# ilyamaclean/microclimf

Hardware: AMD Instinct MI355X
Metric: cell-steps/s (higher is better)
Workload: dtype f64

## Files before the change

### include/mcf.h

```cpp
#ifndef MCF_H
#define MCF_H

#include <stdint.h>

#ifdef __cplusplus
extern "C" {
#endif

#define MCF_ABI_VERSION 8

enum {
    MCF_OUT_TZ = 0,
    MCF_OUT_TLEAF = 1,
    MCF_OUT_RELHUM = 2,
    MCF_OUT_SOILM = 3,
    MCF_OUT_WINDSPEED = 4,
    MCF_OUT_RDIRDOWN = 5,
    MCF_OUT_RDIFDOWN = 6,
    MCF_OUT_RLWDOWN = 7,
    MCF_OUT_RSWUP = 8,
    MCF_OUT_RLWUP = 9,
    MCF_NOUT = 10
};

// ... 138 lines not shown
} mcf_nc_spec;
typedef struct mcf_ncfile mcf_ncfile;
int mcf_nc_create(const char *path, const mcf_nc_spec *spec, mcf_ncfile **nc);
int mcf_nc_write_host(mcf_ncfile *nc, int64_t step0, int64_t nsteps, const double *const vars[MCF_NOUT]);
int mcf_nc_write_plan(mcf_ncfile *nc, mcf_plan *plan, int32_t slot, int64_t slot_step0, int64_t file_step0,
                      int64_t nsteps, float *kernel_ms);
int mcf_nc_close(mcf_ncfile *nc);

int mcf_plan_slot_ptr(mcf_plan *plan, int32_t slot, int32_t var, void **dev_ptr);
typedef struct mcf_ring_layout {
    int32_t tiled;
    int32_t cells_per_tile;
    int32_t block_doubles;
    int32_t slot_days;
    int64_t cells;
    int64_t tile_stride;
    int64_t day_stride;
} mcf_ring_layout;
int mcf_plan_ring_layout(mcf_plan *plan, mcf_ring_layout *layout);
int64_t mcf_ring_index(const mcf_ring_layout *layout, int64_t cell, int64_t step);

int mcf_plan_timer_start(mcf_plan *plan);
int mcf_plan_timer_stop(mcf_plan *plan, float *ms);
int mcf_plan_kernel_timing(mcf_plan *plan, int32_t enable);
int mcf_plan_kernel_stats(mcf_plan *plan, double *total_ms, int64_t *launches);

typedef struct mcf_dispatch_stats {
    int64_t fast_tiles, slow_tiles;
    int64_t irregular_days;
    int64_t fast_launches, slow_launches;
    int64_t canary_trips;
} mcf_dispatch_stats;
int mcf_plan_dispatch_stats(mcf_plan *plan, mcf_dispatch_stats *stats);

#define MCF_NBIO 19
typedef struct mcf_bioclim_sel {
    const int32_t *wetq, *dryq, *hotq, *colq;
    int32_t nwet, ndry, nhot, ncol;
    int32_t air;
    int32_t out[MCF_NBIO];
} mcf_bioclim_sel;
typedef struct mcf_bioclim_out {
    double *bio[MCF_NBIO];
} mcf_bioclim_out;
int mcf_runbioclim1(const mcf_grid_inputs *in, const mcf_options *opt, const mcf_bioclim_sel *sel,
                    mcf_bioclim_out *out);
int mcf_runbioclim2(const mcf_grid_inputs *in, const mcf_options *opt, const mcf_bioclim_sel *sel,
                    mcf_bioclim_out *out);
int mcf_runbioclim3(const mcf_grid_inputs *in, const mcf_options *opt, const mcf_bioclim_sel *sel,
                    mcf_bioclim_out *out);
int mcf_runbioclim4(const mcf_grid_inputs *in, const mcf_options *opt, const mcf_bioclim_sel *sel,
                    mcf_bioclim_out *out);
int mcf_runbioclim1_multi(const mcf_grid_inputs *in, const mcf_options *opt, const mcf_bioclim_sel *sel, const mcf_multi *multi,
                          mcf_bioclim_out *out);
int mcf_runbioclim2_multi(const mcf_grid_inputs *in, const mcf_options *opt, const mcf_bioclim_sel *sel, const mcf_multi *multi,
                          mcf_bioclim_out *out);
int mcf_runbioclim3_multi(const mcf_grid_inputs *in, const mcf_options *opt, const mcf_bioclim_sel *sel, const mcf_multi *multi,
                          mcf_bioclim_out *out);
int mcf_runbioclim4_multi(const mcf_grid_inputs *in, const mcf_options *opt, const mcf_bioclim_sel *sel, const mcf_multi *multi,
                          mcf_bioclim_out *out);

typedef struct mcf_terrain_in {
    int64_t rows, cols;
    int32_t halo_north, halo_south;
    const double *dtm;
    double res;
// ... 216 lines not shown
```

### microclimf_amd/_abi.py

```python
from __future__ import annotations

import ctypes as C
import os
from pathlib import Path

NOUT = 10
OUT_NAMES = ("Tz", "tleaf", "relhum", "soilm", "windspeed", "Rdirdown",
             "Rdifdown", "Rlwdown", "Rswup", "Rlwup")

c_double_p = C.POINTER(C.c_double)
c_int32_p = C.POINTER(C.c_int32)


class Obstime(C.Structure):
    _fields_ = [("year", c_int32_p), ("month", c_int32_p), ("day", c_int32_p),
                ("hour", c_double_p)]


CLIM_FIELDS = ("tc", "es", "ea", "tdew", "pk", "swdown", "difrad", "lwdown",
               "windspeed", "winddir")
POINTM_FIELDS = ("soilm", "Tg", "Tbp", "G", "umu", "kp", "muGp", "dtrp")
VEGP_FIELDS = ("hgt", "pai", "x", "gsmax", "leafr", "leaft", "clump", "leafd",
               "paia", "leafden")
SOILC_FIELDS = ("Smin", "Smax", "gref", "soilb", "Psie", "Vq", "Vm", "Mc", "rho",
# ... 123 lines not shown

class PointSnowOut(C.Structure):
    _fields_ = [(k, c_double_p) for k in POINTSNOW_FIELDS] + [("mxdif", C.c_double), ("iters", C.c_int32)]


class SnowDriverIn(C.Structure):
    _fields_ = [("base", SnowInputs), ("dtm", c_double_p), ("res", C.c_double), ("tfact", C.c_double),
                ("chunk_steps", C.c_int32), ("af_wsa_s", C.c_int32), ("af_wind", c_double_p)]


SNOWDRIVER_OUT = ("Tc", "Tg", "groundsnowdepth", "totalSWE", "snowden")
SnowDriverOut = _ptr_struct("SnowDriverOut", SNOWDRIVER_OUT)


class MicrosnowIn(C.Structure):
    _fields_ = [("grid", C.POINTER(GridInputs)), ("snow", C.POINTER(SnowDriverIn)), ("micro", C.POINTER(SnowInputs)),
                ("mat", C.c_double)]

_PKG_DIR = Path(__file__).resolve().parent
LIB_PATH = _PKG_DIR / "csrc" / "libmcfhip.so"

EXPORTS = (
    "mcf_abi_version", "mcf_last_error", "mcf_device_count",
    "mcf_runmicro1", "mcf_runmicro2", "mcf_runmicro3", "mcf_runmicro4",
    "mcf_plan_create", "mcf_plan_destroy", "mcf_plan_twi_partial",
    "mcf_plan_set_twi_mean", "mcf_plan_upload_forcing_days", "mcf_plan_run_days",
    "mcf_plan_belowground", "mcf_plan_sync", "mcf_plan_fetch", "mcf_plan_fetch_cells", "mcf_plan_fetch_packed", "mcf_plan_slot_ptr",
    "mcf_plan_ring_layout", "mcf_ring_index", "mcf_plan_run_days_at", "mcf_plan_run_days_masked", "mcf_plan_set_mxtc",
    "mcf_snowplan_covered_tiles", "mcf_plan_run_days_cells", "mcf_snowplan_free_cells",
    "mcf_runmicro1_multi", "mcf_runmicro2_multi", "mcf_runmicro3_multi", "mcf_runmicro4_multi", "mcf_plan_fetch_pitched",
    "mcf_snowplan_reset", "mcf_snowplan_checkpoint", "mcf_snowplan_restore", "mcf_snowplan_fetch_cells", "mcf_snowplan_keep_chunk", "mcf_snowplan_can_keep", "mcf_snowplan_set_keep_budget", "mcf_plan_set_mxtc_days", "mcf_snowplan_set_series",
    "mcf_snowplan_release_kept", "mcf_snowplan_meand_accumulate", "mcf_snowplan_micro_setup", "mcf_snowplan_microsnow",
    "mcf_plan_timer_start", "mcf_plan_timer_stop", "mcf_plan_kernel_timing",
    "mcf_plan_kernel_stats", "mcf_plan_dispatch_stats", "mcf_plan_valid_cells", "mcf_plan_bytes", "mcf_selftest_math",
    "mcf_precompute_terrain", "mcf_precompute_terrain_multi", "mcf_runbioclim1_multi", "mcf_runbioclim2_multi",
    "mcf_runbioclim3_multi", "mcf_runbioclim4_multi", "mcf_runbioclim1", "mcf_runbioclim2", "mcf_runbioclim3", "mcf_runbioclim4",
    "mcf_snowenv_from_name", "mcf_gridmodelsnow1", "mcf_gridmodelsnow2", "mcf_gridmicrosnow1",
    "mcf_gridmicrosnow2", "mcf_snowmodel1", "mcf_snowmodel2", "mcf_snowmodel1_multi", "mcf_applycpp3",
    "mcf_snowplan_create", "mcf_snowplan_destroy", "mcf_snowplan_chunks", "mcf_snowplan_surface", "mcf_snowplan_handover", "mcf_snowplan_apply3",
    "mcf_snowplan_surface_partial", "mcf_snowplan_prepare_chunk", "mcf_snowplan_run_chunk", "mcf_snowplan_pack_halo",
    "mcf_snowplan_prepare_chunk_dev",
    "mcf_bigleaf", "mcf_soilm", "mcf_pointmprocess", "mcf_weatherhgt", "mcf_man", "mcf_pointmodelsnow", "mcf_canintfrac", "mcf_meltmu", "mcf_meltmu2", "mcf_tpicalc",
    "mcf_nc_create", "mcf_nc_write_host", "mcf_nc_write_plan", "mcf_nc_close",
    "mcf_flowacc", "mcf_topidx",
    "mcf_runmicrosnow1", "mcf_runmicrosnow2", "mcf_runmicrosnow1_multi", "mcf_snowrun_create", "mcf_snowrun_destroy", "mcf_snowrun_days", "mcf_snowrun_stats", "mcf_snowrun_keep",
    "mcf_snowrun_pass1", "mcf_snowrun_pass2", "mcf_snowplan_run_chunk_pitched", "mcf_snowplan_chunk_af",
    "mcf_plan_create_streamed", "mcf_plan_below_prepare", "mcf_plan_below_set_days", "mcf_below_days_range",
    "mcf_runmicrosnow1_below", "mcf_runmicrosnow1_below_multi", "mcf_snowrun_create_below",
    "mcf_flowacc_device", "mcf_topidx_device", "mcf_plan_create_dtm", "mcf_runmicro_dtm",
)

ABI_VERSION = 8
_lib = None


class McfError(RuntimeError):
    """Raised when libmcfhip reports a non-zero status."""


class DispatchStats(C.Structure):
    _fields_ = [(n, C.c_int64) for n in ("fast_tiles", "slow_tiles", "irregular_days", "fast_launches", "slow_launches",
                                         "canary_trips")]


class RingLayout(C.Structure):
    _fields_ = [("tiled", C.c_int32), ("cells_per_tile", C.c_int32), ("block_doubles", C.c_int32), ("slot_days", C.c_int32),
                ("cells", C.c_int64), ("tile_stride", C.c_int64), ("day_stride", C.c_int64)]
# ... 118 lines not shown
        lib.mcf_plan_below_set_days.argtypes = [P, c_int32_p, C.c_int32]
        lib.mcf_below_days_range.restype = C.c_int
        lib.mcf_below_days_range.argtypes = [c_int32_p, C.c_int32, C.c_int32, C.c_int32, C.c_int32, c_int32_p, c_int32_p]
    lib.mcf_plan_sync.restype = C.c_int
    lib.mcf_plan_sync.argtypes = [P]
    lib.mcf_plan_fetch.restype = C.c_int
    lib.mcf_plan_fetch.argtypes = [P, C.c_int32, C.c_int32, C.c_int64, C.c_int64, c_double_p]
    lib.mcf_plan_fetch_cells.restype = C.c_int
    lib.mcf_plan_fetch_cells.argtypes = [P, C.c_int32, C.c_int32, C.c_int64, C.c_int64, C.POINTER(C.c_int64), C.c_int64,
                                         c_double_p]
    lib.mcf_plan_fetch_packed.restype = C.c_int
    lib.mcf_plan_fetch_packed.argtypes = [P, C.c_int32, C.c_int32, C.c_int64, C.c_int64, C.c_double, c_int32_p,
                                          C.POINTER(C.c_float)]
    lib.mcf_plan_slot_ptr.restype = C.c_int
    lib.mcf_plan_slot_ptr.argtypes = [P, C.c_int32, C.c_int32, C.POINTER(C.c_void_p)]
    try:
        lib.mcf_plan_ring_layout.restype = C.c_int
        lib.mcf_plan_ring_layout.argtypes = [P, C.POINTER(RingLayout)]
        lib.mcf_ring_index.restype = C.c_int64
        lib.mcf_ring_index.argtypes = [C.POINTER(RingLayout), C.c_int64, C.c_int64]
    except AttributeError:
        if "MCF_LIB" not in os.environ:
            raise
    lib.mcf_plan_timer_start.restype = C.c_int
    lib.mcf_plan_timer_start.argtypes = [P]
    lib.mcf_plan_timer_stop.restype = C.c_int
    lib.mcf_plan_timer_stop.argtypes = [P, C.POINTER(C.c_float)]
    lib.mcf_plan_kernel_timing.restype = C.c_int
    lib.mcf_plan_kernel_timing.argtypes = [P, C.c_int32]
    lib.mcf_plan_kernel_stats.restype = C.c_int
    lib.mcf_plan_kernel_stats.argtypes = [P, c_double_p, C.POINTER(C.c_int64)]
    lib.mcf_plan_dispatch_stats.restype = C.c_int
    lib.mcf_plan_dispatch_stats.argtypes = [P, C.POINTER(DispatchStats)]
    lib.mcf_plan_valid_cells.restype = C.c_int64
    lib.mcf_plan_valid_cells.argtypes = [P]
    lib.mcf_plan_bytes.restype = C.c_int64
    lib.mcf_plan_bytes.argtypes = [P]
    lib.mcf_selftest_math.restype = C.c_int
    lib.mcf_selftest_math.argtypes = [C.c_int32, c_double_p, c_double_p, c_double_p, C.c_int64, C.c_int32]
    for fn in (lib.mcf_runbioclim1, lib.mcf_runbioclim2, lib.mcf_runbioclim3, lib.mcf_runbioclim4):
        fn.restype = C.c_int
        fn.argtypes = [GI, OP, C.POINTER(BioclimSel), C.POINTER(BioclimOut)]
    for fn in (lib.mcf_runbioclim1_multi, lib.mcf_runbioclim2_multi, lib.mcf_runbioclim3_multi, lib.mcf_runbioclim4_multi):
        fn.restype = C.c_int
        fn.argtypes = [GI, OP, C.POINTER(BioclimSel), C.POINTER(Multi), C.POINTER(BioclimOut)]
    lib.mcf_snowenv_from_name.restype = C.c_int32
    lib.mcf_snowenv_from_name.argtypes = [C.c_char_p]
    SI = C.POINTER(SnowInputs)
    for fn in (lib.mcf_gridmodelsnow1, lib.mcf_gridmodelsnow2):
        fn.restype = C.c_int
        fn.argtypes = [SI, C.POINTER(SnowModelOut), C.c_int32]
    for fn in (lib.mcf_gridmicrosnow1, lib.mcf_gridmicrosnow2):
        fn.restype = C.c_int
        fn.argtypes = [SI, C.POINTER(Snowm), C.c_double, C.c_double, C.POINTER(C.c_int32 * NOUT), OU, C.c_int32]
    PW, OT = C.POINTER(PointWeather), C.POINTER(Obstime)
    lib.mcf_bigleaf.restype = C.c_int
    lib.mcf_bigleaf.argtypes = [C.c_int64, OT, PW, c_double_p, c_double_p, c_double_p, C.c_double, C.c_double, C.c_double,
                                C.c_double, C.c_int32, C.c_double, C.c_double, C.c_int32, C.POINTER(BigLeafOut)]
    lib.mcf_soilm.restype = C.c_int
    lib.mcf_soilm.argtypes = [C.c_int64, PW] + [C.c_double] * 7 + [c_double_p, C.POINTER(C.c_int64)]
    lib.mcf_pointmprocess.restype = C.c_int
    lib.mcf_pointmprocess.argtypes = [C.c_int64] + [c_double_p] * 7 + [C.c_double] * 7 + [c_double_p] * 6
    lib.mcf_weatherhgt.restype = C.c_int
    lib.mcf_weatherhgt.argtypes = [C.c_int64, OT, PW] + [C.c_double] * 5 + [c_double_p] * 3
    lib.mcf_pointmodelsnow.restype = C.c_int
    lib.mcf_pointmodelsnow.argtypes = [C.c_int64, C.POINTER(Obstime), C.POINTER(PointWeather), c_double_p, c_double_p,
# ... 109 lines not shown
```

### microclimf_amd/api.py

```python
from __future__ import annotations

import ctypes as C
from typing import Mapping, Sequence

import numpy as np

from . import _abi
from .marshal import Marshalled, alloc_outputs, marshal


DTM_DERIVED = ("slope", "aspect", "hor", "svfa", "wsa", "twi")


def dtm_spec(dtm: Mapping, rows: int, cols: int):
    z = np.asfortranarray(np.asarray(dtm["z"], dtype=np.float64))
    hn, hs = int(dtm.get("halo_north", 0)), int(dtm.get("halo_south", 0))
    if z.shape != (hn + rows + hs, cols):
        raise ValueError(f"dtm$z: expected shape {(hn + rows + hs, cols)}, got {z.shape}")
    res = dtm["res"]
    xres, yres = (res, res) if np.isscalar(res) else res
    sp = _abi.DtmSpec()
    sp.dtm = z.ctypes.data_as(_abi.c_double_p)
    sp.halo_north, sp.halo_south = hn, hs
    sp.row0, sp.rows_total = int(dtm.get("row0", 0)), int(dtm.get("rows_total", 0))
# ... 254 lines not shown
    def fetch_packed(self, slot: int, var, step0: int, nsteps: int, scale: float | None = None,
                     timing: bool = False):
        v = _abi.OUT_NAMES.index(var) if isinstance(var, str) else int(var)
        if scale is None:
            scale = self.NC_SCALE[_abi.OUT_NAMES[v]]
        a = np.empty((self.cols, self.rows, nsteps), dtype=np.int32, order="F")
        ms = C.c_float()
        _abi.check(self._lib.mcf_plan_fetch_packed(self._p, slot, v, step0, nsteps, float(scale),
                                                   a.ctypes.data_as(_abi.c_int32_p),
                                                   C.byref(ms) if timing else None))
        return (a, ms.value) if timing else a

    def ring_layout(self) -> dict:
        lay = _abi.RingLayout()
        _abi.check(self._lib.mcf_plan_ring_layout(self._p, C.byref(lay)))
        return {n: int(getattr(lay, n)) for n, _ in lay._fields_}

    def timer_start(self):
        _abi.check(self._lib.mcf_plan_timer_start(self._p))

    def timer_stop(self) -> float:
        ms = C.c_float()
        _abi.check(self._lib.mcf_plan_timer_stop(self._p, C.byref(ms)))
        return ms.value

    def kernel_timing(self, enable: bool = True):
        _abi.check(self._lib.mcf_plan_kernel_timing(self._p, 1 if enable else 0))

    def dispatch_stats(self) -> dict:
        st = _abi.DispatchStats()
        _abi.check(self._lib.mcf_plan_dispatch_stats(self._p, C.byref(st)))
        return {n: int(getattr(st, n)) for n, _ in st._fields_}

    def kernel_stats(self):
        ms, n = C.c_double(), C.c_int64()
        _abi.check(self._lib.mcf_plan_kernel_stats(self._p, C.byref(ms), C.byref(n)))
        return ms.value, n.value


def below_days_range(days, total_days: int, day0: int, ndays: int):
    d = np.ascontiguousarray(np.asarray(days).astype(np.int32))
    pos0, npos = C.c_int32(), C.c_int32()
    _abi.check(_abi.load().mcf_below_days_range(d.ctypes.data_as(_abi.c_int32_p), int(d.size), int(total_days), int(day0), int(ndays),
                                                C.byref(pos0), C.byref(npos)))
    return pos0.value, npos.value


def runbioclim3Cpp(obstime, climdata, pointm, vegp, soilc, reqhgt, zref, lat, lon, Sminp, Smaxp, tfact, mat, out,
                   wetq, dryq, hotq, colq, air, *, device: int = 0, devices=None, n_blocks: int = 0) -> dict:
    return _bioclim("mcf_runbioclim3", False, obstime, climdata, pointm, vegp, soilc, reqhgt, zref, lat, lon,
                    Sminp, Smaxp, tfact, mat, out, wetq, dryq, hotq, colq, air, device, True, devices=devices, n_blocks=n_blocks)


def runbioclim4Cpp(obstime, climdata, pointm, vegp, soilc, reqhgt, zref, lats, lons, Sminp, Smaxp, tfact, mat, out,
                   wetq, dryq, hotq, colq, air, *, device: int = 0, devices=None, n_blocks: int = 0) -> dict:
    return _bioclim("mcf_runbioclim4", True, obstime, climdata, pointm, vegp, soilc, reqhgt, zref, lats, lons,
                    Sminp, Smaxp, tfact, mat, out, wetq, dryq, hotq, colq, air, device, True, devices=devices, n_blocks=n_blocks)
```

### microclimf_amd/csrc/mcf_api.hip

```cpp
#include <hip/hip_runtime.h>
#include <math.h>
#include <stdio.h>
#include <string.h>

#include <algorithm>
#include <chrono>
#include <cstdlib>
#include <future>
#include <memory>
#include <string>
#include <vector>

#include "../../include/mcf.h"
#include "mcf_kernels.h"
#include "mcf_hydro.h"
#include "mcf_terrain.h"
#include "mcf_hostpipe.hpp"
#include "mcf_ncfile.hpp"
#include "mcf_nc4file.hpp"
#include "mcf_rowblocks.hpp"

namespace {

thread_local std::string g_err;
// ... 1429 lines not shown
        HIP_TRY(hipGetLastError());
        mcf::launch_scatter_cells(p->d_celllist, nt_sub, p->d_subring, a.out_tile_stride, slot_base + (int64_t)d * p->ring_day_stride,
                                  p->ring_tile_stride, day_doubles, cpb, nd, p->stream);
        HIP_TRY(hipGetLastError());
    }
    HIP_TRY(hipEventRecord(p->ev_cells_done, p->stream));
    if (trace)
        fprintf(stderr, "[mcf] run_days_cells: %lld cells x %d days; host ms: wait %.3f, class+counts %.3f, offsets+buffers %.3f, enqueue %.3f\n",
                (long long)(n1 + n2), (int)ndays, t1 - t0, t2 - t1, t3 - t2, now() - t3);
    p->cells_inflight = true;
    ++p->cells_runs;
    p->cells_gathered += (n1 + n2) * ndays;
    return MCF_OK;
}

int mcf_plan_dispatch_stats(mcf_plan* p, mcf_dispatch_stats* st) {
    if (!p || !st) return fail(MCF_ERR_ARG, "null argument");
    memset(st, 0, sizeof *st);
    HIP_TRY(hipSetDevice(p->device));
    HIP_TRY(hipStreamSynchronize(p->stream));
    st->fast_tiles = p->fast_enabled ? p->n_fast : 0;
    st->slow_tiles = p->fast_enabled ? p->n_slow : (p->N + p->cpb - 1) / p->cpb;
    for (char c : p->day_irregular) st->irregular_days += c ? 1 : 0;
    st->fast_launches = p->fast_launches;
    st->slow_launches = p->slow_launches;
    if (p->d_fix_count) {
        int32_t v[2] = {0, 0};
        HIP_TRY(hipMemcpy(v, p->d_fix_count, 8, hipMemcpyDeviceToHost));
        st->canary_trips = v[1];
    }
    return MCF_OK;
}

int mcf_plan_belowground(mcf_plan* p) {
    if (!p) return fail(MCF_ERR_ARG, "null plan");
    if (!p->bg) return fail(MCF_ERR_STATE, "reqhgt >= 0: nothing to smooth");
    if (p->bg_stream)
        return fail(MCF_ERR_STATE, "mcf_plan_belowground: a streamed plan leaves the final Tz in each chunk's slot "
                                   "(mcf_plan_below_prepare, then mcf_plan_run_days in day order)");
    if (p->var_slot[MCF_OUT_TZ] < 0) return MCF_OK;
    HIP_TRY(hipSetDevice(p->device));
    mcf::BelowArgs b{};
    b.N = p->N; b.tsteps = (int)p->tsteps; b.complete = p->opt.complete; b.hiy = p->hiy;
    b.per_cell_pointm = p->af ? 1 : 0;
    b.reqhgt = p->opt.reqhgt; b.mat = p->opt.mat;
    b.cellflag_hgt = p->d_veg[0];
    b.tg = p->d_tgser; b.ddsum = p->d_ddsum; b.Tgp = p->d_Tgp; b.Tbp = p->d_Tbp;
    b.scratch = p->d_scratch;
    b.tz = const_cast<double*>(ring_view(p, 0, MCF_OUT_TZ).base);
    if (p->tsteps > (int64_t)p->ring_days * 24)
        return fail(MCF_ERR_STATE, "ring slot smaller than the series");
    mcf::launch_belowground(b, p->stream);
    HIP_TRY(hipGetLastError());
    return MCF_OK;
}

int mcf_plan_sync(mcf_plan* p) {
    if (!p) return fail(MCF_ERR_ARG, "null plan");
    HIP_TRY(hipSetDevice(p->device));
    HIP_TRY(hipStreamSynchronize(p->stream));
    return MCF_OK;
}

int mcf_plan_fetch(mcf_plan* p, int32_t slot, int32_t var, int64_t step0, int64_t nsteps, double* host_dst) {
    return mcf_plan_fetch_pitched(p, slot, var, step0, nsteps, host_dst, 0);
}
// ... 765 lines not shown
```

### microclimf_amd/csrc/mcf_device.hpp

```cpp
#pragma once
#include <hip/hip_runtime.h>
#include <stdint.h>

#include "mcf_kernels.h"


namespace mcf {

constexpr double kPi = 3.14159265358979323846;
constexpr double kToRad = kPi / 180.0;
constexpr double kSb = 5.67e-8;
constexpr double kThetam = 0.365;
constexpr double kKa = 0.4;
constexpr double kOmdy = (2.0 * kPi) / (24.0 * 3600.0);
constexpr uint64_t kNaRealBits = 0x7FF00000000007A2ULL;

enum : int {
    FL_VALID = 1,
    FL_PAI = 2,
    FL_BELOW = 4,
    FL_XONE = 8,
    FL_XINF = 16,
    FL_XZERO = 32,
    FL_ABOVE1 = 64,
    FL_ABOVE2 = 128,
    FL_OMPNAN = 256,
    FL_STOM = 512,
    FL_REGULAR = 1024
};
constexpr int kStepIrregular = 512;
constexpr int kSoilDaily = 1024;

enum CellField : int {
    CF_FLAGS = 0,
    CF_CS, CF_SSCA, CF_SSSA,
    CF_SMIN, CF_RGE, CF_INVRGE, CF_ETA,
    CF_XX, CF_KDENINV,
    CF_PAIT, CF_OM, CF_JDEL, CF_GMA, CF_GMA2, CF_AGM, CF_AGM2, CF_U1, CF_U2, CF_KA1, CF_KA2, CF_KB1, CF_KB2, CF_KG1, CF_KG2, CF_KZ1,
    CF_KZ2, CF_INVD2, CF_GREF, CF_GMAGREF, CF_LOGCLUMP, CF_LOGGI, CF_TRDN, CF_TRDU, CF_AMX,
    CF_PAIAA, CF_ALBD, CF_RDDNG, CF_RDDNZ, CF_RDUPZ, CF_SVFA,
    CF_HOM, CF_HOMP,
    CF_TSV, CF_OMTRDIF,
    CF_UFC, CF_UZFAC, CF_GHAFAC,
    CF_ABSPSIE, CF_INVSMAX, CF_SOILB, CF_RHO, CF_CSA, CF_C1, CF_C1MC4, CF_C3,
    CF_GSMAX, CF_RSMX, CF_INV02RSMX, CF_RAT, CF_RATC, CF_PSIW0, CF_KK, CF_MUDENINV,
    CF_PAI, CF_OMPC, CF_KSAT, CF_PSUNSAT, CF_SHADEFAC,
    CF_OML1, CF_OML2,
    CF_EMG, CF_EMA, CF_INVLEAFD,
    CF_A2H, CF_INTHH, CF_INTHZ, CF_HGT, CF_INVHGT, CF_INVHMZ, CF_NEARFAC, CF_LEAFDEN, CF_OMEMPAI,
    CF_SINLAT, CF_COSLAT, CF_COSB, CF_SINB,
    CF_CROWPOS, CF_CCOLPOS,
    CF_ELEVD, CF_PKFAC,
    CF_COUNT
};
constexpr int kCellDirs = 32;

enum TimeField : int {
    TF_TC = 0, TF_ES, TF_EA, TF_TDEW, TF_PK, TF_RSW, TF_RDIF, TF_RLW, TF_U2,
    TF_SOILMP, TF_GP, TF_UMU, TF_KP, TF_MUGP, TF_DTRP,
    TF_CZ, TF_SZ, TF_CAZ, TF_SAZ, TF_TANSA, TF_ZEND,
    TF_COSC, TF_TAN2C, TF_TANC, TF_INV2COSC,
    TF_TAN2B, TF_TANB, TF_INV2COSB,
    TF_DE, TF_GHRRAD, TF_REM, TF_LAPK, TF_MUPM, TF_INVMUPM, TF_WFAC, TF_GFAC,
    TF_RBEAM, TF_RB,
// ... 1362 lines not shown
```

### microclimf_amd/csrc/mcf_kernels.h

```cpp
#pragma once
#include <hip/hip_runtime.h>
#include <stdint.h>

namespace mcf {

struct Globals {
    double reqhgt;
    double reqhgt2;
    double zref;
    double dTmx;
    double hf0p;
    double hf500p;
    int shadowmask;
};

#define RING_BLOCK(cpb) ((((cpb) * 24 + 63) / 64) * 64)
__host__ __device__ inline int ring_block_doubles(int cpb) { return RING_BLOCK(cpb); }
__host__ __device__ inline int ring_pos(int cpb, int cell, int hour) {
    if (cpb == 21) {
        const int w = hour / 3, hh = hour - 3 * w;
        return 64 * w + (cell < 16 ? 16 * hh + cell : 48 + 5 * hh + (cell - 16));
    }
    return hour * cpb + cell;
}
// ... 202 lines not shown
    int32_t* dst;
};
void launch_pack_nc(const PackNcArgs& a, int64_t nsteps, hipStream_t s);
void launch_pack_transpose(const RingView& src, int64_t step0, int64_t rows, int64_t cols, int64_t nsteps, double scale,
                           int32_t* dst, hipStream_t s);
void launch_twi_partial(const double* twi, int64_t n, double tfact, double* out2, hipStream_t s);
int twi_scratch_doubles();
void launch_cell_setup(const CellSetupArgs& a, hipStream_t s);
void launch_time_setup(const TimeSetupArgs& a, hipStream_t s);
void launch_date_setup(const DateSetupArgs& a, hipStream_t s);
void launch_mxtc(const double* tc, int64_t N, int nsteps, double* mx, hipStream_t s);
void launch_solve(const SolveArgs& a, int cells_per_block, bool af, bool bg, bool fast, bool soil_daily, hipStream_t s);
void launch_solve_bg_tiled(const SolveArgs& a, int cells_per_block, bool af, hipStream_t s);
void launch_tile_regular(const double* cellc, int64_t N, int layers, int cpb, uint8_t* out, hipStream_t s);
void launch_cells_class(const uint8_t* need, const uint8_t* tile_regular, int64_t N, int cpb, uint8_t* cls, int32_t* blockcnt,
                        hipStream_t s);
void launch_cells_place(const uint8_t* cls, int64_t N, const int32_t* blockoff, int32_t* list, hipStream_t s);
void launch_gather_image(const int32_t* list, int64_t ntiles_sub, const double* src, int64_t ntiles_src, int layers, int cpb,
                         double* dst, hipStream_t s);
void launch_scatter_cells(const int32_t* list, int64_t ntiles_sub, const double* sub, int64_t sub_tile_stride, double* ring,
                          int64_t tile_stride, int64_t day_doubles, int cpb, int ndays, hipStream_t s);
void launch_belowground(const BelowArgs& a, hipStream_t s);
void launch_selftest_math(int kind, const double* x, const double* y, double* out, int64_t n, hipStream_t s);

}
struct mcf_plan;
namespace mcf {
int plan_ring_views(mcf_plan* p, int slot, RingView views[10], int32_t has[10], hipStream_t* stream, int64_t* N, int* device,
                    int* slot_days);

int cell_field_count();
void print_variant_stats();
int soil_daily_bit();
int step_irregular_bit();
int time_field_count();
double hf_pow02(double rs);

}
```

### microclimf_amd/csrc/mcf_kernels.hip

```cpp
#include <hip/hip_runtime.h>
#include <math.h>
#include <stdio.h>
#include <stdint.h>
#include <algorithm>

#include "mcf_device.hpp"
#include "mcf_kernels.h"

#ifndef MCF_WAVES_PER_EU
#define MCF_WAVES_PER_EU 4
#endif
#ifndef MCF_AF_WAVES
#define MCF_AF_WAVES 3
#endif

namespace mcf {

__global__ void k_fill(double* __restrict__ p, int64_t n, double v) {
    int64_t i = (int64_t)blockIdx.x * blockDim.x + threadIdx.x;
    int64_t stride = (int64_t)gridDim.x * blockDim.x;
    for (; i < n; i += stride) p[i] = v;
}

__global__ void k_gather_cells(RingView src, int64_t step0, int64_t nsteps, const int64_t* __restrict__ cells,
// ... 304 lines not shown
    {
        bool dirs_ok = true;
        for (int d = 0; d < 24; ++d) { const double v = a.hor[(int64_t)d * N + c]; out[(CF_COUNT + d) * cpb] = v; dirs_ok = dirs_ok && isfinite(v); }
        for (int d = 0; d < 8; ++d) { const double v = a.wsa[(int64_t)d * N + c]; out[(CF_COUNT + 24 + d) * cpb] = v; dirs_ok = dirs_ok && !isinf(v); }
        const bool bare = pai == 0.0 && hgt == 0.0;
        const bool veg = pai > 0.0 && hgt > 0.0 && clump >= 0.0 && clump < 1.0 && a.leafd[c] > 0.0 && isfinite(x) && x > 0.0;
        const bool soil = Smin >= 0.0 && Smax > Smin && a.gsmax[c] >= 0.0 && a.g.zref > 0.0;
        const bool below = (flags & FL_BELOW) != 0;
        const bool fields = fin[0] && (veg ? fin[1] : true) && (below ? fin[2] : fin[3]);
        if (dirs_ok && soil && (bare || veg) && fields) flags |= FL_REGULAR;
    }
    put(CF_FLAGS, (double)flags);
}

__global__ __launch_bounds__(256) void k_time_setup(TimeSetupArgs a) {
    int k = blockIdx.x * blockDim.x + threadIdx.x;
    if (k >= a.nsteps) return;
    TimeVals t;
    for (int f = 0; f < 15; ++f) t.v[f] = a.raw[f][k];
    SolDate sd = sol_date(a.year[k], a.month[k], a.day[k]);
    SolPos sp = sol_site(sd, a.hour[k], sin(a.lat * kPi / 180.0), cos(a.lat * kPi / 180.0), a.lon);
    derive_time(t, sp, dir_index(a.winddir[k], 45.0, 8));
    int dy = k / 24, hr = k % 24;
    {
        const double* sm = a.raw[TF_SOILMP] + dy * 24;
        bool daily = true;
        for (int h = 1; h < 24; ++h) daily = daily && sm[h] == sm[0];
        if (daily) t.v[TF_IDX] = (double)((int)t.v[TF_IDX] | kSoilDaily);
    }
    double* dst = a.tt + ((int64_t)dy * TF_COUNT) * 24 + hr;
    for (int f = 0; f < TF_COUNT; ++f) dst[f * 24] = t.v[f];
}

__global__ __launch_bounds__(256) void k_date_setup(DateSetupArgs a) {
    int k = blockIdx.x * blockDim.x + threadIdx.x;
    if (k >= a.nsteps) return;
    SolDate sd = sol_date(a.year[k], a.month[k], a.day[k]);
    const double A = 0.261799 * (a.hour[k] + sd.eot / 60.0 - 12.0);
    a.dt[4 * (int64_t)k + 0] = sd.sindec;
    a.dt[4 * (int64_t)k + 1] = sd.cosdec;
    a.dt[4 * (int64_t)k + 2] = cos(A);
    a.dt[4 * (int64_t)k + 3] = sin(A);
    a.windex[k] = dir_index(a.winddir[k], 45.0, 8);
}

__global__ __launch_bounds__(256) void k_mxtc(const double* __restrict__ tc, int64_t N, int nsteps,
                                              double* __restrict__ mx) {
    int64_t c = (int64_t)blockIdx.x * blockDim.x + threadIdx.x;
    if (c >= N) return;
    double m = mx[c];
    for (int k = 0; k < nsteps; ++k) {
        double v = tc[c + N * k];
        if (v > m) m = v;
    }
    mx[c] = m;
}

__global__ __launch_bounds__(256) void k_mxtc_coarse(const double* __restrict__ force, int64_t stride, int crows, int ccols,
                                                     int nsteps, const double* __restrict__ rowpos,
                                                     const double* __restrict__ colpos, int64_t rows, int64_t N,
                                                     int altcorrect, const double* __restrict__ elevd,
                                                     const double* __restrict__ pkfac, double* __restrict__ mx) {
    int64_t c = (int64_t)blockIdx.x * blockDim.x + threadIdx.x;
    if (c >= N) return;
    const CoarseTap tap(rowpos[c % rows], colpos[c / rows], crows, ccols);
    const int64_t cN = (int64_t)crows * ccols;
// ... 12 lines not shown
        if (v > m) m = v;
    }
    mx[c] = m;
}

constexpr int solve_threads(int cpb) { return ((cpb * 24 + 63) / 64) * 64; }
static_assert(solve_threads(21) == 512 && solve_threads(32) == 768, "ring_block_doubles() must agree");

template <int CPB, int AF, int BG, bool F, bool SSREQ>
__device__ __forceinline__ void solve_tile(const SolveArgs& a, const int64_t tile, const int day0, const int ndays, const int rot) {
    constexpr int NT = solve_threads(CPB);
    static_assert(NT == RING_BLOCK(CPB), "tile-day block = one value per lane");
    constexpr int IMG = (int)tile_image_doubles_dev(CPB);
    __shared__ __attribute__((aligned(256))) double s_tile[IMG];
    double* const s_cell = s_tile;
    __shared__ double s_time[AF ? 1 : 3 * TF_COUNT * 24];
    constexpr bool PRE = CPB == 21;
    __shared__ double s_ext[3][3][CPB];
    __shared__ double s_dd[BG ? 24 * CPB : 1];
    constexpr bool SS = SSREQ && (AF == 0) && (2 * CPB <= 64);
    __shared__ double s_soil[SS ? 3 * SD_COUNT * CPB : 1];
    __shared__ int s_trip;
    constexpr bool CLDS = (AF == 2) && SSREQ;
    constexpr int CU_ROWS = 4, CU_F = 15, CU_SLOT = CU_ROWS * CU_F * 24;
    __shared__ double s_cu[CLDS ? 2 * 2 * CU_SLOT : 1];
    __shared__ double s_cw[2];
    __shared__ int s_ci[9];

    const int tid = threadIdx.x;
    int cl = tid % CPB;
    bool lane_on = tid < CPB * 24;
    int hr;
    uint32_t pos;
    if (CPB == 21) {
        const int w = tid >> 6, l = tid & 63;
        if (l < 48) { cl = l & 15; hr = 3 * w + (l >> 4); }
        else { const int j = l - 48; cl = 16 + (j % 5); hr = 3 * w + (j / 5); lane_on = j < 15; if (!lane_on) { cl = 20; hr = 3 * w + 2; } }
        hr = hr + 6 * rot;
        hr -= hr >= 24 ? 24 : 0;
        pos = (uint32_t)(64 * (hr / 3) + l);
    } else if (CPB == 32) {
        const int wave = tid >> 6;
        const int tab = ((wave & 3) == 0) ? (wave == 0 ? 12 : wave == 4 ? 16 : 20)
                      : ((wave & 3) == 1) ? (wave == 1 ? 10 : wave == 5 ? 6 : 2)
                      : ((wave & 3) == 2) ? (wave == 2 ? 14 : wave == 6 ? 18 : 22)
                                          : (wave == 3 ? 8 : wave == 7 ? 4 : 0);
        hr = tab + ((tid >> 5) & 1);
        pos = (uint32_t)(hr * 32 + cl);
    } else {
        hr = tid / CPB;
        if (hr > 23) hr = 23;
        pos = (uint32_t)tid;
    }
    uint32_t posb = pos * 8u;
    const int64_t N = a.N;
    const int64_t c0 = tile * CPB;
    const int64_t c = c0 + cl;
    const bool in_grid = lane_on && c < N;

    auto image_of = [&](int layer) { return reinterpret_cast<const double2*>(a.cellc + ((int64_t)layer * a.ntiles_total + tile) * IMG); };
    auto stage_cells = [&](int layer) {
        const double2* src = image_of(layer);
        double2* dst = reinterpret_cast<double2*>(s_tile);
        for (int q = tid; q < IMG / 2; q += NT) dst[q] = src[q];
    };
    const CellLds<CPB> C{s_cell + cl};
    int flags = 0;
    bool valid = false;
    int cur_layer = a.daylayer ? a.daylayer[day0] : 0;
    __shared__ double s_exptab[256];
    __shared__ __attribute__((aligned(16))) double s_logtab[512];
// ... 105 lines not shown
            const uint64_t mb = __builtin_amdgcn_ballot_w64(brk), mh = __builtin_amdgcn_ballot_w64(have && tid < 32);
            const int nk = 64 - __builtin_clzll(mh | 1ull);
            const int b = mb ? __builtin_ctzll(mb) : nk;
            if (tid < 2) {
                const int fk = tid ? (b < nk ? b : 0) : 0, lk = tid ? nk - 1 : b - 1;
                const double rpf = s_cell[CF_CROWPOS * CPB + fk], rpl = s_cell[CF_CROWPOS * CPB + lk], cpx = s_cell[CF_CCOLPOS * CPB + fk];
                const int rb = (int)floor(rpf), re = (int)floor(rpl) + 1;
                const int cc0 = (int)floor(cpx), cc1 = cc0 + 1 < a.ccols ? cc0 + 1 : cc0;
                int nr = (re < a.crows ? re : a.crows - 1) - rb + 1;
                if (tid == 1 && b >= nk) nr = 0;
                s_ci[4 * tid + 0] = rb; s_ci[4 * tid + 1] = nr < CU_ROWS ? nr : CU_ROWS; s_ci[4 * tid + 2] = cc0; s_ci[4 * tid + 3] = cc1;
                s_cw[tid] = cpx - floor(cpx);
                if (tid == 0) s_ci[8] = b;
            }
        }
        __syncthreads();
        double v0, v1;
        stage_issue(day0, 0, v0, v1);
        stage_commit(day0, 0, v0, v1);
        __syncthreads();
    }
    enter_layer(day0);
    double* ring_day = BG == 1 ? nullptr : a.out_base + tile * a.out_tile_stride + (int64_t)a.slot_day0 * a.out_day_stride;
    double* tg_day = (BG == 2 && a.tg_ring) ? a.tg_ring + tile * a.tg_tile_stride : nullptr;
    for (int dl = 0; dl < ndays; ++dl, ++run) {
        const int dabs = day0 + dl;
        const int layer = a.daylayer ? a.daylayer[dabs] : 0;
        if (layer != cur_layer) {
            __syncthreads();
            if (layer >= 0) stage_cells(layer);
            __syncthreads();
            cur_layer = layer;
            enter_layer(dabs);
        }
        const int64_t kl = (int64_t)(dabs - a.day0) * 24 + hr;
        uint64_t osel = a.out_sel;
        asm volatile("" : "+s"(osel));
        double* lin = nullptr;
        if (BG == 1) lin = a.out_base + (c + N * (a.slot_step0 + kl));
        auto put = [&](int v, double val) {
            const unsigned sel = (unsigned)(osel >> (4 * v)) & 15u;
            if (sel == 15u) return;
            if (BG == 1) { if (in_grid) lin[(int64_t)sel * a.out_stride] = val; }
            else {
                asm("" : "+v"(posb));
                *(double*)((char*)ring_day + ((size_t)sel * (NT * 8)) + posb) = val;
            }
        };
        constexpr int TPER = (TF_COUNT * 24 + NT - 1) / NT;
        double pre[TPER];
        const bool stage = !AF && dl + 1 < ndays;
        if (stage) {
            const double* src = a.tt + (int64_t)(dabs + 1) * TF_COUNT * 24;
#pragma unroll
            for (int i = 0; i < TPER; ++i) {
                int q = tid + i * NT;
                pre[i] = src[q < TF_COUNT * 24 ? q : TF_COUNT * 24 - 1];
            }
        }
        double cs0 = 0.0, cs1 = 0.0;
        if (CLDS && dl + 1 < ndays) stage_issue(dabs + 1, (run + 1) & 1, cs0, cs1);
        TimeVals tv;
        const double* fday = (AF == 1) ? a.af_base + tile * a.af_tile_stride + (int64_t)(dabs - a.day0) * a.af_day_stride : nullptr;
        auto force = [&](int f, unsigned pb) { return *(const double*)((const char*)fday + (size_t)f * (NT * 8) + pb); };
        if (AF && valid) {
            const int64_t kabs = (int64_t)dabs * 24 + hr;
// ... 95 lines not shown
            asm("v_max_f64 %0, %0, %1" : "+v"(tmx3) : "v"(t1));
            asm("v_max_f64 %0, %0, %1" : "+v"(tmx3) : "v"(t2));
            asm("v_min_f64 %0, %0, %1" : "+v"(tmn3) : "v"(t1));
            asm("v_min_f64 %0, %0, %1" : "+v"(tmn3) : "v"(t2));
            asm("v_max_f64 %0, %0, %1" : "+v"(rmx3) : "v"(r1));
            asm("v_max_f64 %0, %0, %1" : "+v"(rmx3) : "v"(r2));
            if (valid && (l < 16 || (l >= 48 && l < 53))) {
                double (*ext)[CPB] = s_ext[run % 3];
                __hip_atomic_fetch_max(&ext[0][cl], tmx3, __ATOMIC_RELAXED, __HIP_MEMORY_SCOPE_WORKGROUP);
                __hip_atomic_fetch_min(&ext[1][cl], tmn3, __ATOMIC_RELAXED, __HIP_MEMORY_SCOPE_WORKGROUP);
                __hip_atomic_fetch_max(&ext[2][cl], rmx3, __ATOMIC_RELAXED, __HIP_MEMORY_SCOPE_WORKGROUP);
            }
        }
        if (CLDS && dl + 1 < ndays) stage_commit(dabs + 1, (run + 1) & 1, cs0, cs1);
        if (stage) {
            double* dst = s_time + ((run + 1) % 3) * (TF_COUNT * 24);
#pragma unroll
            for (int i = 0; i < TPER; ++i) {
                int q = tid + i * NT;
                if (q < TF_COUNT * 24) dst[q] = pre[i];
            }
        }
        __syncthreads();
        if (tid < 3 * CPB)
            s_ext[(run + 2) % 3][tid / CPB][tid % CPB] = tid < CPB ? -999.0 : tid < 2 * CPB ? 999.0 : -999.9;
        if (SS) {
            if ((tid >> 6) == (run & 7) % (NT / 64) && dl + 2 < ndays) produce_soil(day0 + dl + 2, run + 2);
        }
        if (valid && a.need_pass2) {
            const double tmx = s_ext[run % 3][0][cl], tmn = s_ext[run % 3][1][cl], Rmx = s_ext[run % 3][2][cl];
            const double dtr = tmx - tmn;
            Pass2Out p2{};
            if (AF) derive_time_af_pass2(tv);
            if (AF) pass2<F, false>(C, TR, SL, g, flags, dTcap, cy, dtr, Rmx, need_tv, p2, MK, cn);
            else pass2<F, SS>(C, TL, SL, g, flags, dTcap, cy, dtr, Rmx, need_tv, p2, MK, cn);
            if (BG == 1) {
                a.tgser[c + N * ((int64_t)dabs * 24 + hr)] = p2.Tg;
                s_dd[hr * CPB + cl] = p2.DD;
            } else if (BG == 2) {
                *(double*)((char*)tg_day + posb) = p2.Tg;
                s_dd[hr * CPB + cl] = p2.DD;
            } else {
                const bool pos_h = g.reqhgt > 0.0;
                put(0, pos_h ? p2.Tz : p2.Tg);
                put(1, pos_h ? p2.tleaf : NA);
                put(2, pos_h ? p2.rh : NA);
                put(7, p2.lwdn);
                put(9, p2.lwup);
            }
        } else if (BG != 1 || in_grid) {
            if (!BG) put(0, NA);
            if (BG == 2 && tg_day) *(double*)((char*)tg_day + posb) = 0.0;
            put(1, NA);
            put(2, NA);
            put(7, NA);
            put(9, NA);
        }
        if (BG) {
            if (valid && (BG == 1 || a.need_pass2)) {
                put(1, NA);
                put(2, NA);
                put(7, NA);
                put(9, NA);
            }
            if (BG == 1 || a.ddsum) {
                __syncthreads();
                if (valid && hr == 0) {
                    double s = 0.0;
// ... 771 lines not shown
        const int64_t n = std::min<int64_t>(65535, nsteps - k0);
        dim3 grid((unsigned)((src.N + 255) / 256), (unsigned)n);
        hipLaunchKernelGGL(k_untile, grid, dim3(256), 0, s, src, step0 + k0, dst + src.N * k0);
    }
}
void launch_mxtc_coarse(const double* force, int64_t stride, int crows, int ccols, int tsteps, const double* rowpos,
                        const double* colpos, int64_t rows, int64_t N, int altcorrect, const double* elevd,
                        const double* pkfac, double* mx, hipStream_t s) {
    hipLaunchKernelGGL(k_mxtc_coarse, dim3((unsigned)((N + 255) / 256)), dim3(256), 0, s, force, stride, crows, ccols, tsteps,
                       rowpos, colpos, rows, N, altcorrect, elevd, pkfac, mx);
}
void launch_gather_cells(const RingView& src, int64_t step0, int64_t nsteps, const int64_t* cells, int64_t ncells, double* dst,
                         hipStream_t s) {
    const int64_t n = ncells * nsteps;
    if (n <= 0) return;
    hipLaunchKernelGGL(k_gather_cells, dim3((unsigned)((n + 255) / 256)), dim3(256), 0, s, src, step0, nsteps, cells, ncells, dst);
}
void launch_fill(double* p, int64_t n, double v, hipStream_t s) {
    if (n <= 0) return;
    int64_t blocks = (n + 255) / 256;
    if (blocks > 65536) blocks = 65536;
    hipLaunchKernelGGL(k_fill, dim3((unsigned)blocks), dim3(256), 0, s, p, n, v);
}
void launch_twi_partial(const double* twi, int64_t n, double tfact, double* out2, hipStream_t s) {
    hipLaunchKernelGGL(k_twi_partial, dim3(kTwiParts), dim3(256), 0, s, twi, n, tfact, out2);
    hipLaunchKernelGGL(k_twi_finish, dim3(1), dim3(64), 0, s, out2);
}
void launch_cell_setup(const CellSetupArgs& a, hipStream_t s) {
    hipLaunchKernelGGL(k_cell_setup, dim3((unsigned)((a.N + 255) / 256)), dim3(256), 0, s, a);
}
void launch_time_setup(const TimeSetupArgs& a, hipStream_t s) {
    if (a.nsteps <= 0) return;
    hipLaunchKernelGGL(k_time_setup, dim3((unsigned)((a.nsteps + 255) / 256)), dim3(256), 0, s, a);
}
void launch_date_setup(const DateSetupArgs& a, hipStream_t s) {
    if (a.nsteps <= 0) return;
    hipLaunchKernelGGL(k_date_setup, dim3((unsigned)((a.nsteps + 255) / 256)), dim3(256), 0, s, a);
}
void launch_mxtc(const double* tc, int64_t N, int nsteps, double* mx, hipStream_t s) {
    hipLaunchKernelGGL(k_mxtc, dim3((unsigned)((N + 255) / 256)), dim3(256), 0, s, tc, N, nsteps, mx);
}
void launch_belowground(const BelowArgs& a, hipStream_t s) {
    hipLaunchKernelGGL(k_belowground, dim3((unsigned)((a.N + 63) / 64)), dim3(64), 0, s, a);
}

static dim3 solve_grid(int64_t ntiles) { return dim3((unsigned)(8 * ((ntiles + 7) / 8))); }
void launch_below_dd(const BelowDDArgs& a, hipStream_t s) {
    if (a.N <= 0 || a.ndays <= 0) return;
    hipLaunchKernelGGL(k_below_dd, dim3((unsigned)((a.N + 255) / 256)), dim3(256), 0, s, a);
}
void launch_below_acc(const BelowStreamArgs& a, hipStream_t s) {
    if (a.N <= 0 || a.ndays_chunk <= 0) return;
    hipLaunchKernelGGL(k_below_acc, dim3((unsigned)((a.N + 255) / 256)), dim3(256), 0, s, a);
}
void launch_below_finish(const BelowStreamArgs& a, hipStream_t s) {
    if (a.N <= 0) return;
    hipLaunchKernelGGL(k_below_finish, dim3((unsigned)((a.N + 255) / 256)), dim3(256), 0, s, a);
}
void launch_below_chunk(const BelowStreamArgs& a, hipStream_t s) {
    const int days = a.ndays_chunk + (a.tail ? 1 : 0);
    if (a.N <= 0 || days <= 0) return;
    hipLaunchKernelGGL(k_below_chunk, dim3((unsigned)((a.N + 255) / 256), (unsigned)days), dim3(256), 0, s, a);
    if (a.complete && a.ndays_chunk > 0)
        hipLaunchKernelGGL(k_below_carry, dim3((unsigned)((a.N + 255) / 256)), dim3(256), 0, s, a);
}
template <int CPB>
// ... 77 lines not shown
static void launch_solve_coarse(SolveArgs a, bool bg, bool fast, bool lds, hipStream_t s) {
    constexpr int CPB = 32;
    if (a.ntiles_launch <= 0) {
        a.ntiles_launch = (a.N + CPB - 1) / CPB;
        a.tile_list = nullptr;
    }
    const dim3 grid = solve_grid(a.ntiles_launch), block(solve_threads(CPB));
    if (bg) hipLaunchKernelGGL((k_solve<CPB, 2, true, false, false>), grid, block, 0, s, a);
    else if (fast) {
        if (lds) hipLaunchKernelGGL((k_solve<CPB, 2, false, true, true>), grid, block, 0, s, a);
        else hipLaunchKernelGGL((k_solve<CPB, 2, false, true, false>), grid, block, 0, s, a);
        hipLaunchKernelGGL((k_solve_fix<CPB, 2>), dim3(512), block, 0, s, a);
    } else hipLaunchKernelGGL((k_solve<CPB, 2, false, false, false>), grid, block, 0, s, a);
}
int twi_scratch_doubles() { return 2 + 2 * kTwiParts; }
int cell_field_count() { return CF_COUNT; }
int step_irregular_bit() { return kStepIrregular; }
int time_field_count() { return TF_COUNT; }
double hf_pow02(double rs) {
    double Hlf = 1.09767 * pow(rs, 0.2672778);
    double Hf = -1.0 / (1.0 + exp(2.0 - Hlf));
    return pow(fabs(Hf), 0.2);
}

void launch_solve(const SolveArgs& a, int cells_per_block, bool af, bool bg, bool fast, bool soil_daily, hipStream_t s) {
    if (a.N <= 0 || a.ndays <= 0) return;
    if (a.crows > 0) { launch_solve_coarse(a, bg, fast, soil_daily, s); return; }
    if (cells_per_block == 32) launch_solve_cpb<32>(a, af, bg, fast, soil_daily, s);
    else if (cells_per_block == 21) launch_solve_cpb<21>(a, af, bg, fast, soil_daily, s);
    else if (cells_per_block == 42) launch_solve_cpb<42>(a, af, bg, fast, soil_daily, s);
    else launch_solve_cpb<16>(a, af, bg, fast, soil_daily, s);
}
int soil_daily_bit() { return kSoilDaily; }
void print_variant_stats() {}

}
```

Baseline: 30.91 billion.

## Shift per-day hour-to-wave mapping to align daylight with wavefront groups

Adds a per-day hour shift (0-2), computed on device from shortwave radiation and stored in the time-index field. In the CPB=21 fast path, each lane then remaps its hour and ring position so that daylit hours are packed into fewer 3-hour wavefront groups. The aim is to cut the number of wavefronts that run the expensive daylight branch. The cost is an extra small kernel per time setup, some extra register and bitfield work per step, and hf0p and hf500p globals reloaded from the kernarg segment.

```diff
diff --git a/include/mcf.h b/include/mcf.h
--- a/include/mcf.h
+++ b/include/mcf.h
@@ -194,6 +194,7 @@
     int64_t canary_trips;
 } mcf_dispatch_stats;
 int mcf_plan_dispatch_stats(mcf_plan *plan, mcf_dispatch_stats *stats);
+int mcf_plan_hour_shifts(mcf_plan *plan, int32_t *shifts, int32_t ndays);
 
 #define MCF_NBIO 19
 typedef struct mcf_bioclim_sel {
diff --git a/microclimf_amd/_abi.py b/microclimf_amd/_abi.py
--- a/microclimf_amd/_abi.py
+++ b/microclimf_amd/_abi.py
@@ -179,7 +179,7 @@
     "mcf_snowplan_reset", "mcf_snowplan_checkpoint", "mcf_snowplan_restore", "mcf_snowplan_fetch_cells", "mcf_snowplan_keep_chunk", "mcf_snowplan_can_keep", "mcf_snowplan_set_keep_budget", "mcf_plan_set_mxtc_days", "mcf_snowplan_set_series",
     "mcf_snowplan_release_kept", "mcf_snowplan_meand_accumulate", "mcf_snowplan_micro_setup", "mcf_snowplan_microsnow",
     "mcf_plan_timer_start", "mcf_plan_timer_stop", "mcf_plan_kernel_timing",
-    "mcf_plan_kernel_stats", "mcf_plan_dispatch_stats", "mcf_plan_valid_cells", "mcf_plan_bytes", "mcf_selftest_math",
+    "mcf_plan_kernel_stats", "mcf_plan_dispatch_stats", "mcf_plan_hour_shifts", "mcf_plan_valid_cells", "mcf_plan_bytes", "mcf_selftest_math",
     "mcf_precompute_terrain", "mcf_precompute_terrain_multi", "mcf_runbioclim1_multi", "mcf_runbioclim2_multi",
     "mcf_runbioclim3_multi", "mcf_runbioclim4_multi", "mcf_runbioclim1", "mcf_runbioclim2", "mcf_runbioclim3", "mcf_runbioclim4",
     "mcf_snowenv_from_name", "mcf_gridmodelsnow1", "mcf_gridmodelsnow2", "mcf_gridmicrosnow1",
@@ -364,6 +364,8 @@
     lib.mcf_plan_kernel_stats.argtypes = [P, c_double_p, C.POINTER(C.c_int64)]
     lib.mcf_plan_dispatch_stats.restype = C.c_int
     lib.mcf_plan_dispatch_stats.argtypes = [P, C.POINTER(DispatchStats)]
+    lib.mcf_plan_hour_shifts.restype = C.c_int
+    lib.mcf_plan_hour_shifts.argtypes = [P, c_int32_p, C.c_int32]
     lib.mcf_plan_valid_cells.restype = C.c_int64
     lib.mcf_plan_valid_cells.argtypes = [P]
     lib.mcf_plan_bytes.restype = C.c_int64
diff --git a/microclimf_amd/api.py b/microclimf_amd/api.py
--- a/microclimf_amd/api.py
+++ b/microclimf_amd/api.py
@@ -310,6 +310,11 @@
         _abi.check(self._lib.mcf_plan_dispatch_stats(self._p, C.byref(st)))
         return {n: int(getattr(st, n)) for n, _ in st._fields_}
 
+    def hour_shifts(self, ndays: int) -> np.ndarray:
+        s = np.zeros(int(ndays), dtype=np.int32)
+        _abi.check(self._lib.mcf_plan_hour_shifts(self._p, s.ctypes.data_as(_abi.c_int32_p), int(ndays)))
+        return s
+
     def kernel_stats(self):
         ms, n = C.c_double(), C.c_int64()
         _abi.check(self._lib.mcf_plan_kernel_stats(self._p, C.byref(ms), C.byref(n)))
diff --git a/microclimf_amd/csrc/mcf_api.hip b/microclimf_amd/csrc/mcf_api.hip
--- a/microclimf_amd/csrc/mcf_api.hip
+++ b/microclimf_amd/csrc/mcf_api.hip
@@ -1485,6 +1485,21 @@
     return MCF_OK;
 }
 
+int mcf_plan_hour_shifts(mcf_plan* p, int32_t* shifts, int32_t ndays) {
+    if (!p || !shifts) return fail(MCF_ERR_ARG, "null argument");
+    if (p->af) return fail(MCF_ERR_STATE, "mcf_plan_hour_shifts: array forcing has no hour shift");
+    if (ndays != p->ndays) return fail(MCF_ERR_ARG, "mcf_plan_hour_shifts: ndays is not the plan's number of days");
+    if (ndays <= 0) return MCF_OK;
+    HIP_TRY(hipSetDevice(p->device));
+    const int tfc = mcf::time_field_count();
+    std::vector<double> idx((size_t)ndays);
+    HIP_TRY(hipMemcpy2DAsync(idx.data(), 8, p->d_tt + (int64_t)(tfc - 1) * 24, (size_t)tfc * 24 * 8, 8, (size_t)ndays,
+                             hipMemcpyDeviceToHost, p->stream));
+    HIP_TRY(hipStreamSynchronize(p->stream));
+    for (int d = 0; d < ndays; ++d) shifts[d] = mcf::hour_shift_of((int)idx[(size_t)d]);
+    return MCF_OK;
+}
+
 int mcf_plan_belowground(mcf_plan* p) {
     if (!p) return fail(MCF_ERR_ARG, "null plan");
     if (!p->bg) return fail(MCF_ERR_STATE, "reqhgt >= 0: nothing to smooth");
diff --git a/microclimf_amd/csrc/mcf_device.hpp b/microclimf_amd/csrc/mcf_device.hpp
--- a/microclimf_amd/csrc/mcf_device.hpp
+++ b/microclimf_amd/csrc/mcf_device.hpp
@@ -30,6 +30,8 @@
 };
 constexpr int kStepIrregular = 512;
 constexpr int kSoilDaily = 1024;
+constexpr int kHourShiftBit = 11;
+constexpr int kHourShiftMask = 3 << kHourShiftBit;
 
 enum CellField : int {
     CF_FLAGS = 0,
diff --git a/microclimf_amd/csrc/mcf_kernels.h b/microclimf_amd/csrc/mcf_kernels.h
--- a/microclimf_amd/csrc/mcf_kernels.h
+++ b/microclimf_amd/csrc/mcf_kernels.h
@@ -258,6 +258,7 @@
 int cell_field_count();
 void print_variant_stats();
 int soil_daily_bit();
+int hour_shift_of(int idx);
 int step_irregular_bit();
 int time_field_count();
 double hf_pow02(double rs);
diff --git a/microclimf_amd/csrc/mcf_kernels.hip b/microclimf_amd/csrc/mcf_kernels.hip
--- a/microclimf_amd/csrc/mcf_kernels.hip
+++ b/microclimf_amd/csrc/mcf_kernels.hip
@@ -360,6 +360,24 @@
     for (int f = 0; f < TF_COUNT; ++f) dst[f * 24] = t.v[f];
 }
 
+__global__ __launch_bounds__(256) void k_hour_shift(double* tt, int ndays) {
+    const int d = blockIdx.x * blockDim.x + threadIdx.x;
+    if (d >= ndays) return;
+    double* const row = tt + (int64_t)d * TF_COUNT * 24;
+    const double* const rsw = row + TF_RSW * 24;
+    double* const idx = row + TF_IDX * 24;
+    int first = -1, runs = 0;
+    bool prev = false, irregular = false;
+    for (int h = 0; h < 24; ++h) {
+        const bool lit = rsw[h] > 0.0;
+        if (lit && !prev) { ++runs; if (first < 0) first = h; }
+        prev = lit;
+        irregular = irregular || (((int)idx[h] & kStepIrregular) != 0);
+    }
+    const int s = (runs == 1 && !irregular) ? first % 3 : 0;
+    idx[0] = (double)(((int)idx[0] & ~kHourShiftMask) | (s << kHourShiftBit));
+}
+
 __global__ __launch_bounds__(256) void k_date_setup(DateSetupArgs a) {
     int k = blockIdx.x * blockDim.x + threadIdx.x;
     if (k >= a.nsteps) return;
@@ -438,11 +456,23 @@
     bool lane_on = tid < CPB * 24;
     int hr;
     uint32_t pos;
+    constexpr bool HS = CPB == 21 && AF == 0 && !BG && F;
+    uint32_t hs_hr = 0, hs_pos = 0;
     if (CPB == 21) {
         const int w = tid >> 6, l = tid & 63;
         if (l < 48) { cl = l & 15; hr = 3 * w + (l >> 4); }
         else { const int j = l - 48; cl = 16 + (j % 5); hr = 3 * w + (j / 5); lane_on = j < 15; if (!lane_on) { cl = 20; hr = 3 * w + 2; } }
         hr = hr + 6 * rot;
+        if (HS) {
+#pragma unroll
+            for (int sh = 2; sh >= 0; --sh) {
+                int h = hr + sh;
+                h -= h >= 24 ? 24 : 0;
+                const uint32_t ps = lane_on ? (uint32_t)ring_pos(21, cl, h) : (uint32_t)(64 * (h / 3) + 63);
+                hs_hr = (hs_hr << 5) | (uint32_t)h;
+                hs_pos = (hs_pos << 9) | ps;
+            }
+        }
         hr -= hr >= 24 ? 24 : 0;
         pos = (uint32_t)(64 * (hr / 3) + l);
     } else if (CPB == 32) {
@@ -614,6 +644,15 @@
             __syncthreads();
             cur_layer = layer;
             enter_layer(dabs);
+        }
+        if (HS) {
+            int iv = (int)s_time[(run % 3) * (TF_COUNT * 24) + TF_IDX * 24];
+            asm volatile("" : "+v"(iv));
+            uint32_t sft = (uint32_t)__builtin_amdgcn_readfirstlane(iv);
+            asm volatile("" : "+s"(sft));
+            sft = (sft >> kHourShiftBit) & 3u;
+            hr = (int)__builtin_amdgcn_ubfe(hs_hr, 5u * sft, 5u);
+            posb = __builtin_amdgcn_ubfe(hs_pos, 9u * sft, 9u) * 8u;
         }
         const int64_t kl = (int64_t)(dabs - a.day0) * 24 + hr;
         uint64_t osel = a.out_sel;
@@ -775,8 +814,19 @@
             const double dtr = tmx - tmn;
             Pass2Out p2{};
             if (AF) derive_time_af_pass2(tv);
-            if (AF) pass2<F, false>(C, TR, SL, g, flags, dTcap, cy, dtr, Rmx, need_tv, p2, MK, cn);
-            else pass2<F, SS>(C, TL, SL, g, flags, dTcap, cy, dtr, Rmx, need_tv, p2, MK, cn);
+            Globals g2;
+            const Globals* gq = &g;
+            if (HS) {
+                g2 = g;
+                gq = &g2;
+                typedef const __attribute__((address_space(4))) char* kptr;
+                kptr ka = (kptr)__builtin_amdgcn_kernarg_segment_ptr();
+                asm volatile("" : "+s"(ka));
+                g2.hf0p = *(const __attribute__((address_space(4))) double*)(ka + offsetof(SolveArgs, g) + offsetof(Globals, hf0p));
+                g2.hf500p = *(const __attribute__((address_space(4))) double*)(ka + offsetof(SolveArgs, g) + offsetof(Globals, hf500p));
+            }
+            if (AF) pass2<F, false>(C, TR, SL, *gq, flags, dTcap, cy, dtr, Rmx, need_tv, p2, MK, cn);
+            else pass2<F, SS>(C, TL, SL, *gq, flags, dTcap, cy, dtr, Rmx, need_tv, p2, MK, cn);
             if (BG == 1) {
                 a.tgser[c + N * ((int64_t)dabs * 24 + hr)] = p2.Tg;
                 s_dd[hr * CPB + cl] = p2.DD;
@@ -1614,6 +1664,8 @@
 void launch_time_setup(const TimeSetupArgs& a, hipStream_t s) {
     if (a.nsteps <= 0) return;
     hipLaunchKernelGGL(k_time_setup, dim3((unsigned)((a.nsteps + 255) / 256)), dim3(256), 0, s, a);
+    const int ndays = a.nsteps / 24;
+    if (ndays > 0) hipLaunchKernelGGL(k_hour_shift, dim3((unsigned)((ndays + 255) / 256)), dim3(256), 0, s, a.tt, ndays);
 }
 void launch_date_setup(const DateSetupArgs& a, hipStream_t s) {
     if (a.nsteps <= 0) return;
@@ -1757,6 +1809,7 @@
     else launch_solve_cpb<16>(a, af, bg, fast, soil_daily, s);
 }
 int soil_daily_bit() { return kSoilDaily; }
+int hour_shift_of(int idx) { return (idx & kHourShiftMask) >> kHourShiftBit; }
 void print_variant_stats() {}
 
 }
diff --git a/microclimf_amd/hourshift.py b/microclimf_amd/hourshift.py
--- /dev/null
+++ b/microclimf_amd/hourshift.py
@@ -0,0 +1,37 @@
+import numpy as np
+
+
+def _days(swdown):
+    sw = np.asarray(swdown, dtype=np.float64)
+    nd = sw.size // 24
+    return sw[: nd * 24].reshape(nd, 24)
+
+
+def hour_shifts(swdown, irregular_day=None) -> np.ndarray:
+    lit = _days(swdown) > 0.0
+    nd = lit.shape[0]
+    rises = lit & ~np.concatenate([np.zeros((nd, 1), dtype=bool), lit[:, :-1]], axis=1)
+    runs = rises.sum(axis=1)
+    first = np.where(lit.any(axis=1), lit.argmax(axis=1), 0)
+    s = np.where(runs == 1, first % 3, 0).astype(np.int32)
+    if irregular_day is not None:
+        s[np.asarray(irregular_day, dtype=bool)[:nd]] = 0
+    return s
+
+
+def day_path_waves(swdown, shifts=None) -> np.ndarray:
+    lit = _days(swdown) > 0.0
+    nd = lit.shape[0]
+    s = np.zeros(nd, dtype=np.int64) if shifts is None else np.asarray(shifts, dtype=np.int64)
+    hours = (s[:, None, None] + 3 * np.arange(8)[None, :, None] + np.arange(3)[None, None, :]) % 24
+    return np.take_along_axis(lit[:, None, :].repeat(8, axis=1), hours, axis=2).any(axis=2).sum(axis=1)
+
+
+def summary(swdown, irregular_day=None) -> dict:
+    lit = _days(swdown) > 0.0
+    s = hour_shifts(swdown, irregular_day)
+    fixed, shifted = day_path_waves(swdown), day_path_waves(swdown, s)
+    return {"days": int(lit.shape[0]), "daylight_hours": float(lit.sum(axis=1).mean()),
+            "fixed": float(fixed.mean()), "shifted": float(shifted.mean()), "lane_bound": float(lit.sum(axis=1).mean() / 3.0),
+            "saved_wave_days_per_tile_day": float((fixed - shifted).mean()),
+            "shift_counts": [int((s == v).sum()) for v in (0, 1, 2)]}
```

Result: no change. 30.76 billion (-0.5%).
